# itsdfish/DifferentialEvolutionMCMC.jl

Measured on AMD Instinct MI355X. Metric: particle-updates/sec (proposal+loglike+accept) at D=32, N=1e5, higher is better.
Workload: dtype f64; 1 GPU; cfg3: MvNormal full-Sigma D=32, N=100000 obs, n_groups=256x1, Np=256, sampler defaults, schedule=two_colour, loglike=direct; particles_per_gpu=65536, parallelism=groups sharded x1, one all-gather per migration

## Files before the change

### differentialevolutionmcmc.jl_amd/csrc/demc_kernels.hpp

```cpp
#pragma once
#include <type_traits>
#include "demc_device.hpp"

namespace demc {

enum Family : int {
    FAM_GAUSSIAN = 0, FAM_MVN_ISO = 1, FAM_MVN_FULL = 2, FAM_BINOMIAL = 3, FAM_HIER_BINOMIAL = 4,
    FAM_HIER_GAUSSIAN = 5, FAM_LBA = 6, FAM_LNR = 7, FAM_RASTRIGIN = 8, FAM_USER = 100
};
enum Mode : int { MODE_STEP = 0, MODE_IDENT = 1 };

struct DimTab {
    double lo, hi;
    double a, b;
    double c;
    int kind, ref;
};

struct DimSeg {
    int start, pad;
    DimTab t;
    double pad2;
};
constexpr int kMaxDimSeg = 16;
// ... 1453 lines not shown
                        if (c0 < d) a_ = fma(tr[c0] - xb0, y0, a_);
                        if (c1 < d) a_ = fma(tr[c1] - xb1, y1, a_);
                        if (p.sx)
                            s_ = fma(y1, sx1, y0 * sx0);
                        else {
                            const int qr = q_lo + pass * ppp + wrow0 + pr;
                            if (qr < q_hi) {
                                double* yrow = STREAM ? ybuf + (size_t)(qr - q_lo) * p.dpad
                                                      : p.Ypad + ((size_t)g * Np + p.a_lo + qr) * p.dpad;
                                if (c0 < p.dpad) yrow[c0] = y0;
                                if (c1 < p.dpad) yrow[c1] = y1;
                            }
                        }
                        a_ = subgroup_sum(a_, 16);
                        s_ = subgroup_sum(s_, 16);
                        if (row == 0) {
                            tr[D] = a_;
                            tr[D + 1] = s_;
                        }
                    }
                }
                __builtin_amdgcn_fence(__ATOMIC_RELEASE, "wavefront");
                __builtin_amdgcn_wave_barrier();
                aux = th[D];
                S = th[D + 1];
            } else
            for (int k = sl; 2 * k < d; k += lpp) {
                const int c0 = 2 * k, c1 = 2 * k + 1;
                double y0 = 0.0, y1 = 0.0;
                const double* ainv_g = ld_ainv ? (const double*)ainv_s : p.Ainv;
                if (p.Ainv) {
                    if (c1 < d) {
#pragma unroll 4
                        for (int j = 0; j < d; ++j) {
                            const double t = th[j] - xb_s[j];
                            y0 = fma(ainv_g[j * d + c0], t, y0);
                            y1 = fma(ainv_g[j * d + c1], t, y1);
                        }
                    } else
                        for (int j = 0; j < d; ++j) y0 = fma(ainv_g[j * d + c0], th[j] - xb_s[j], y0);
                } else {
                    y0 = th[c0] - xb_s[c0];
                    if (c1 < d) y1 = th[c1] - xb_s[c1];
                }
                aux = fma(th[c0] - xb_s[c0], y0, aux);
                if (c1 < d) aux = fma(th[c1] - xb_s[c1], y1, aux);
                if (p.sx) {
                    S = fma(y0, p.sx[c0], S);
                    if (c1 < d) S = fma(y1, p.sx[c1], S);
                } else if (valid) {
                    double* yrow = STREAM ? ybuf + (size_t)srow * p.dpad : p.Ypad + slot * p.dpad;
                    yrow[c0] = y0;
                    if (c1 < p.dpad) yrow[c1] = (c1 < d) ? y1 : 0.0;
                }
            }
            if (!p.sx && valid && !PREP_MFMA && !STREAM)
                for (int c = 2 * ((d + 1) / 2) + sl; c < p.dpad; c += lpp) p.Ypad[slot * p.dpad + c] = 0.0;
            if (!PREP_MFMA) {
                aux = group_sum(aux, lpp, s_gsum);
                S = group_sum(S, lpp, s_gsum);
            }
        }

        if (pass == DEMC_STAMP_PASS || n_pass == 1) DEMC_STAMP(7);
        if (FUSE_OBS) {
            __builtin_amdgcn_fence(__ATOMIC_RELEASE, "wavefront");
            __builtin_amdgcn_wave_barrier();
            if (lpp > 64) __syncthreads();
            S = group_sum(obs_range_sum(p, scr + srow * scr_stride, sl, p.N, lpp), lpp, s_gsum);
        }

        if (!p.fuse_accept) {
            if (sl == 0 && valid) {
                p.prop_prior[slot] = prior;
                p.prop_oob[slot] = oob ? 1 : 0;
                p.prop_adj[slot] = adj;
                if (FUSE_PREP) {
                    p.aux[slot] = aux;
                    if (p.sx) p.partial[slot] = S;
                }
                if (!PLAIN && p.trace) {
                    p.tr_idx[slot * 4 + 0] = kind;
                    p.tr_idx[slot * 4 + 1] = i0;
                    p.tr_idx[slot * 4 + 2] = i1;
                    p.tr_idx[slot * 4 + 3] = i2;
                }
            }
            __builtin_amdgcn_fence(__ATOMIC_RELEASE, "wavefront");
            __builtin_amdgcn_wave_barrier();
            if (lpp > 64 && use_scr) __syncthreads();
            continue;
        }

        if (STREAM) {
            if (sl == 0 && valid) {
                double* tr = scr + srow * scr_stride;
                tr[D] = aux; tr[D + 2] = prior; tr[D + 3] = (double)oob; tr[D + 4] = adj; tr[D + 5] = u_acc;
                if (!PLAIN && p.trace && wr_hbm) {
                    p.tr_idx[slot * 4 + 0] = kind; p.tr_idx[slot * 4 + 1] = i0;
                    p.tr_idx[slot * 4 + 2] = i1; p.tr_idx[slot * 4 + 3] = i2;
                }
            }
            continue;
        }
        if (pass == DEMC_STAMP_PASS || n_pass == 1) DEMC_STAMP(8);
        finish_particle(valid, pl, slot, pt, srow, prior, oob, adj, aux, S, u_acc, kind, i0, i1, i2);
        __builtin_amdgcn_fence(__ATOMIC_RELEASE, "wavefront");
        __builtin_amdgcn_wave_barrier();
        if (lpp > 64 && use_scr) __syncthreads();
        if (pass == DEMC_STAMP_PASS || n_pass == 1) DEMC_STAMP(9);
    }
    if (STREAM) {
        __syncthreads();
        DEMC_STAMP(16);
        const int n_act = q_hi - q_lo;
        {
            const int nw = WG / 64;
            const int nt = xt_hi - xt_lo, per_w = (nt + nw - 1) / nw;
            const int t_lo = wave * per_w < nt ? wave * per_w : nt, t_hi = t_lo + per_w < nt ? t_lo + per_w : nt;
            lds_ptr outw = (lds_ptr)(part_l + (size_t)wave * p.st_nact_max);
            if (p.st_x_lds)
                cross_stage<lds_cptr>((lds_cptr)ybuf, p.dpad, n_act, (lds_cptr)xs, t_lo, t_hi, p.st_chunk_tiles, outw, lane);
            else
                cross_stage<glb_cptr>((lds_cptr)ybuf, p.dpad, n_act, (glb_cptr)(p.Xf + (size_t)xt_lo * (p.dpad >> 2) * 64), t_lo, t_hi,
                                      p.n_tiles - xt_lo, outw, lane);
        }
        __syncthreads();
        DEMC_STAMP(17);
        const unsigned epoch = (unsigned)(step + 1);
        unsigned long long* gran = p.st_gran + (((size_t)(step & 1) * p.n_groups + gi) * p.st_C) * p.st_nact_max * 2;
        if (tid < n_act) {
            double v = 0.0;
            for (int wv = 0; wv < WG / 64; ++wv) v += part_l[(size_t)wv * p.st_nact_max + tid];
            unsigned long long* mine = gran + ((size_t)c_idx * p.st_nact_max + tid) * 2;
            store_granule(mine, epoch, (unsigned)__double2loint(v));
            store_granule(mine + 1, epoch, (unsigned)__double2hiint(v));
        }
        DEMC_STAMP(18);
        {
            const int tot = p.st_C * n_act * 2;
            unsigned spins = 0;
            for (;;) {
                int ok = 1;
                for (int e = tid; e < tot; e += WG) {
                    const int cc = e / (2 * n_act), r = e - cc * 2 * n_act;
                    const unsigned long long x = load_granule(gran + (size_t)cc * p.st_nact_max * 2 + r);
                    ok &= (unsigned)(x >> 32) == epoch;
                    part_c[(size_t)cc * p.st_nact_max * 2 + r] = (unsigned)x;
                }
                if (__syncthreads_and(ok)) break;
                if (++spins > (1u << 22)) {
                    if (tid == 0) *p.st_err = 1u;
                    break;
                }
                __builtin_amdgcn_s_sleep(2);
            }
        }
        DEMC_STAMP(19);
        if (tid < n_act) {
            double S = 0.0;
            for (int cc = 0; cc < p.st_C; ++cc) {
                const unsigned* h2 = part_c + ((size_t)cc * p.st_nact_max + tid) * 2;
                S += __hiloint2double((int)h2[1], (int)h2[0]);
            }
            scr[tid * scr_stride + D + 1] = S;
        }
        __syncthreads();
        for (int pass = 0; pass < n_pass; ++pass) {
            const int q = q_lo + pass * ppp + sub;
            const bool valid = q < q_hi;
            const int pl = p.a_lo + (valid ? q : q_lo);
            const size_t slot = (size_t)g * Np + pl;
            const int srow = pass * ppp + sub;
            const double* tr = scr + (valid ? srow : 0) * scr_stride;
            finish_particle(valid, pl, slot, rows + (size_t)pl * D, valid ? srow : 0, tr[D + 2], (int)tr[D + 3], tr[D + 4], tr[D],
                            tr[D + 1], tr[D + 5], 0, -1, -1, -1);
        }
        DEMC_STAMP(20);
    }
    if (RES) __syncthreads();
    DEMC_STAMP(10);
    }
}

#define DEMC_K1_PHASE_INSTANCES(X) \
    X(256, false, TAIL_NONE, false, 0, false) X(256, false, TAIL_PREP, false, 0, false) \
    X(256, false, TAIL_PREP_MFMA, false, 0, false) X(256, false, TAIL_OBS, false, 0, false) \
    X(256, true, TAIL_NONE, false, 0, false) X(256, true, TAIL_PREP, false, 0, false) \
    X(256, true, TAIL_PREP_MFMA, false, 0, false) X(256, true, TAIL_OBS, false, 0, false) \
    X(256, true, TAIL_NONE, false, 1, false) X(256, true, TAIL_PREP, false, 1, false) \
    X(256, true, TAIL_PREP_MFMA, false, 1, false) X(256, true, TAIL_OBS, false, 1, false) \
    X(512, false, TAIL_NONE, false, 0, false) X(512, false, TAIL_PREP, false, 0, false) \
    X(512, false, TAIL_PREP_MFMA, false, 0, false) X(512, false, TAIL_OBS, false, 0, false) \
    X(256, true, TAIL_NONE, false, 2, false) X(256, true, TAIL_PREP, false, 2, false) \
    X(256, true, TAIL_PREP_MFMA, false, 2, false) X(256, true, TAIL_OBS, false, 2, false) \
    X(256, false, TAIL_NONE, false, 1, false) X(256, false, TAIL_PREP, false, 1, false) \
    X(256, false, TAIL_PREP_MFMA, false, 1, false) X(256, false, TAIL_OBS, false, 1, false) \
    X(256, false, TAIL_NONE, false, 2, false) X(256, false, TAIL_PREP, false, 2, false) \
    X(256, false, TAIL_PREP_MFMA, false, 2, false) X(256, false, TAIL_OBS, false, 2, false)
#define DEMC_K1_RES_INSTANCES(X) \
    X(256, true, TAIL_NONE, true, 0, false) X(256, true, TAIL_PREP, true, 0, false) \
    X(256, true, TAIL_PREP_MFMA, true, 0, false) X(256, true, TAIL_OBS, true, 0, false) \
    X(512, true, TAIL_NONE, true, 0, false) X(512, true, TAIL_PREP, true, 0, false) \
    X(512, true, TAIL_PREP_MFMA, true, 0, false) X(512, true, TAIL_OBS, true, 0, false) \
    X(256, true, TAIL_NONE, true, 1, false) X(256, true, TAIL_PREP, true, 1, false) \
    X(256, true, TAIL_PREP_MFMA, true, 1, false) X(256, true, TAIL_OBS, true, 1, false) \
    X(512, true, TAIL_NONE, true, 1, false) X(512, true, TAIL_PREP, true, 1, false) \
    X(512, true, TAIL_PREP_MFMA, true, 1, false) X(512, true, TAIL_OBS, true, 1, false) \
    X(256, true, TAIL_NONE, true, 2, false) X(256, true, TAIL_PREP, true, 2, false) \
    X(256, true, TAIL_PREP_MFMA, true, 2, false) X(256, true, TAIL_OBS, true, 2, false) \
    X(512, true, TAIL_NONE, true, 2, false) X(512, true, TAIL_PREP, true, 2, false) \
    X(512, true, TAIL_PREP_MFMA, true, 2, false) X(512, true, TAIL_OBS, true, 2, false)
#define DEMC_K1_STREAM_INSTANCES(X) \
    X(256, true, TAIL_PREP, true, 0, true) X(256, true, TAIL_PREP_MFMA, true, 0, true) \
    X(256, true, TAIL_PREP, true, 1, true) X(256, true, TAIL_PREP_MFMA, true, 1, true) \
    X(256, true, TAIL_PREP, true, 2, true) X(256, true, TAIL_PREP_MFMA, true, 2, true) \
    X(512, true, TAIL_PREP, true, 0, true) X(512, true, TAIL_PREP_MFMA, true, 0, true) \
    X(512, true, TAIL_PREP, true, 1, true) X(512, true, TAIL_PREP_MFMA, true, 1, true) \
    X(512, true, TAIL_PREP, true, 2, true) X(512, true, TAIL_PREP_MFMA, true, 2, true)
#ifdef DEMC_K1_EXTERN
#define DEMC_X_(...) extern template __global__ void k_propose<__VA_ARGS__>(KParams);
DEMC_K1_PHASE_INSTANCES(DEMC_X_)
DEMC_K1_RES_INSTANCES(DEMC_X_)
DEMC_K1_STREAM_INSTANCES(DEMC_X_)
#undef DEMC_X_
#endif

template <int KS, int MT>
__global__ __launch_bounds__(256, 2) void k_cross_mfma(KParams p, const double* __restrict__ Ypad, int dpad, int k0,
                                                       const double* __restrict__ Xf, int n_tiles, int n_chunks,
                                                       int part0) {
    const int lane = threadIdx.x & 63, wave = threadIdx.x >> 6;
    const int chunk = blockIdx.x % n_chunks;
    const int ptile = blockIdx.x / n_chunks;
    const int n_prop = p.n_groups * p.n_act;
    const int q0 = (ptile * 4 + wave) * (MT * 16);
    const int ksx = dpad >> 2;

    double a[MT][KS];
#pragma unroll
    for (int mt = 0; mt < MT; ++mt) {
        const int q = q0 + mt * 16 + (lane & 15);
        const bool ok = q < n_prop;
        const size_t slot = ok ? (size_t)slot_of(p, q) : 0;
        const double* yrow = Ypad + slot * dpad + k0 + (lane >> 4);
#pragma unroll
        for (int ks = 0; ks < KS; ++ks) {
            const double v = yrow[4 * ks];
            a[mt][ks] = ok ? v : 0.0;
        }
    }
    d4 acc[MT];
#pragma unroll
    for (int mt = 0; mt < MT; ++mt) acc[mt] = (d4){0.0, 0.0, 0.0, 0.0};

    const int per = (n_tiles + n_chunks - 1) / n_chunks;
    const int t0 = chunk * per, t1 = (t0 + per < n_tiles) ? t0 + per : n_tiles;
    const size_t tstride = (size_t)ksx * 64;
    const double* xb = Xf + (size_t)(k0 >> 2) * 64 + lane;
    double b0[KS], b1[KS];
    {
        const double* x = xb + (size_t)(t0 < t1 ? t0 : n_tiles) * tstride;
#pragma unroll
        for (int ks = 0; ks < KS; ++ks) b0[ks] = x[ks * 64];
    }
    for (int t = t0; t < t1; t += 2) {
        {
            const double* x = xb + (size_t)(t + 1 < t1 ? t + 1 : n_tiles) * tstride;
#pragma unroll
            for (int ks = 0; ks < KS; ++ks) b1[ks] = x[ks * 64];
        }
#pragma unroll
        for (int ks = 0; ks < KS; ++ks)
#pragma unroll
            for (int mt = 0; mt < MT; ++mt)
                acc[mt] = __builtin_amdgcn_mfma_f64_16x16x4f64(a[mt][ks], b0[ks], acc[mt], 0, 0, 0);
        {
            const double* x = xb + (size_t)(t + 2 < t1 ? t + 2 : n_tiles) * tstride;
#pragma unroll
            for (int ks = 0; ks < KS; ++ks) b0[ks] = x[ks * 64];
        }
#pragma unroll
        for (int ks = 0; ks < KS; ++ks)
#pragma unroll
            for (int mt = 0; mt < MT; ++mt)
                acc[mt] = __builtin_amdgcn_mfma_f64_16x16x4f64(a[mt][ks], b1[ks], acc[mt], 0, 0, 0);
    }
#pragma unroll
    for (int mt = 0; mt < MT; ++mt)
#pragma unroll
        for (int r = 0; r < 4; ++r) {
            double v = acc[mt][r];
            v += __shfl_xor(v, 1);
            v += __shfl_xor(v, 2);
            v += __shfl_xor(v, 4);
            v += __shfl_xor(v, 8);
            const int q = q0 + mt * 16 + (lane >> 4) + 4 * r;
            if ((lane & 15) == 0 && q < n_prop) p.partial[(size_t)(part0 + chunk) * p.P + slot_of(p, q)] = v;
        }
}
#define DEMC_CROSS_INSTANCES(X) X(1, 4) X(2, 4) X(4, 4) X(8, 4) X(16, 4)

template <int DP>
__global__ __launch_bounds__(256) void k_direct_mvn(KParams p, int n_chunks, unsigned long long* __restrict__ clk) {
    int pblock = blockIdx.x, chunk = blockIdx.y;
    if ((n_chunks & 7) == 0) {
        const unsigned lin = blockIdx.y * gridDim.x + blockIdx.x, xcd = lin & 7u, j = lin >> 3;
        chunk = (int)((j / gridDim.x) * 8u + xcd);
        pblock = (int)(j % gridDim.x);
    }
    const int q = pblock * 256 + threadIdx.x;
    const int n_prop = p.n_groups * p.n_act;
    const bool ok = q < n_prop;
    const size_t slot = ok ? (size_t)slot_of(p, q) : 0;
    double m[DP];
    const double* mrow = p.Ypad + slot * p.dpad;
#pragma unroll
    for (int k = 0; k < DP; ++k) m[k] = (ok && k < p.d) ? mrow[k] : 0.0;
    const long long per = (p.N + n_chunks - 1) / n_chunks;
    const long long i0 = chunk * per, i1 = (i0 + per < p.N) ? i0 + per : p.N;
    double acc[4] = {0.0, 0.0, 0.0, 0.0};
    const double* z = p.data + i0 * DP;
    for (long long i = i0; i < i1; ++i, z += DP) {
#pragma unroll
        for (int k = 0; k < DP; k += 4) {
#pragma unroll
            for (int e = 0; e < 4; ++e) {
                const double r = z[k + e] - m[k + e];
                acc[e] = fma(r, r, acc[e]);
            }
        }
    }
    if (ok) p.partial[(size_t)chunk * p.P + slot] = (acc[0] + acc[1]) + (acc[2] + acc[3]);
    if (clk) {
        const unsigned long long t1 = __builtin_amdgcn_s_memtime(), r1 = __builtin_amdgcn_s_memrealtime();
        const unsigned xcc = __builtin_amdgcn_s_getreg(20 | (3 << 11)) & 15u;
        const unsigned hwid = __builtin_amdgcn_s_getreg(4 | (31 << 11));
        if (threadIdx.x == 0) {
            const size_t wg = (size_t)blockIdx.y * gridDim.x + blockIdx.x;
            clk[3 * wg] = t1;
            clk[3 * wg + 1] = r1;
            clk[3 * wg + 2] = (xcc << 8) | ((hwid >> 8) & 0xffu);
        }
    }
}
#define DEMC_DIRECT_INSTANCES(X) X(8) X(16) X(32) X(64)

#ifndef DEMC_DEVICE_HELPERS_ONLY
__global__ __launch_bounds__(256) void k_obs_loglike(KParams p, int n_chunks) {
    constexpr int kTabPhi = kPhiIntervals * kPhiRow, kTabErfcx = kLogPhiRows * kLogPhiRow;
    __shared__ double s_tab[kTabPhi > kTabErfcx ? kTabPhi : kTabErfcx];
    if (p.family == FAM_LBA) {
        for (int i = threadIdx.x; i < kTabPhi; i += 256) s_tab[i] = kPhiTable[i];
        __syncthreads();
    } else if (p.family == FAM_LNR) {
        for (int i = threadIdx.x; i < kTabErfcx; i += 256) s_tab[i] = kLogPhiTable[i];
        __syncthreads();
    }
    const int q = blockIdx.x * 256 + threadIdx.x;
    const int n_prop = p.n_groups * p.n_act;
    const int chunk = blockIdx.y;
    if (q >= n_prop) return;
    const size_t slot = (size_t)slot_of(p, q);
    const double* th = p.prop + slot * p.D;
    const long long per = (p.N + n_chunks - 1) / n_chunks;
    const long long i0 = chunk * per, i1 = (i0 + per < p.N) ? i0 + per : p.N;
    double acc;
    if (p.family == FAM_LBA)
        acc = p.n_acc == 3 ? lba_range_sum<3>(p, th, i0, i1, 1, s_tab)
              : p.n_acc == 2 ? lba_range_sum<2>(p, th, i0, i1, 1, s_tab) : lba_range_sum<0>(p, th, i0, i1, 1, s_tab);
    else if (p.family == FAM_LNR)
        acc = lnr_range_sum(p, th, i0, i1, 1, s_tab);
    else
        acc = obs_range_sum(p, th, i0, i1, 1);
    p.partial[(size_t)chunk * p.P + slot] = acc;
}
#endif

#ifndef DEMC_DEVICE_HELPERS_ONLY
template <int NA>
__global__ __launch_bounds__(256, 2) void k_lba_wave(KParams p, int n_chunks, unsigned long long* __restrict__ clk) {
    __shared__ double s_tab[kPhiIntervals * kPhiRow];
    for (int i = threadIdx.x; i < kPhiIntervals * kPhiRow; i += 256) s_tab[i] = kPhiTable[i];
    __syncthreads();
    const int lane = threadIdx.x & 63, wave = __builtin_amdgcn_readfirstlane(threadIdx.x >> 6);
    const int q = blockIdx.x * 4 + wave;
    const int n_prop = p.n_groups * p.n_act;
    const int chunk = blockIdx.y;
    if (q >= n_prop) return;
    const size_t slot = (size_t)slot_of(p, q);
    const double* th = p.prop + slot * p.D;
    const int na = NA > 0 ? NA : p.n_acc;
    double nu[8], nuS[8];
#pragma unroll
    for (int a = 0; a < 8; ++a) {
        nu[a] = a < na ? th[a] : 0.0;
        nuS[a] = kPhiS * nu[a];
    }
    const double A = th[na], kk = th[na + 1], tau = th[na + 2], b = A + kk, inv_A = 1.0 / A;
    const double kS = kPhiS * kk, bS = kPhiS * b, inv_SA = inv_A * (1.0 / kPhiS);
    double pneg = 1.0;
#pragma unroll
    for (int a = 0; a < (NA > 0 ? NA : 8); ++a)
        if (a < na) {
            double qq, Ph;
            phiS_Phi_table(s_tab, -nuS[a], qq, Ph);
            pneg *= Ph;
        }
    const double inv_norm = 1.0 / (1.0 - pneg);
    constexpr long long kStep = 64LL * kLbaBatch;
    const long long n_steps = (p.N + kStep - 1) / kStep, per = (n_steps + n_chunks - 1) / n_chunks;
    const long long i0 = (long long)chunk * per * kStep, i1r = i0 + per * kStep, i1 = i1r < p.N ? i1r : p.N;
    double acc = 0.0;
    long long base = i0;
    for (; base + kStep <= i1; base += kStep) {
        double cc[kLbaBatch], rr[kLbaBatch];
#pragma unroll
        for (int j = 0; j < kLbaBatch; ++j) {
            cc[j] = p.data[base + 64LL * j + lane];
            rr[j] = p.data2[base + 64LL * j + lane];
        }
        double prod = 1.0;
#pragma unroll
        for (int j = 0; j < kLbaBatch; ++j)
            prod *= lba_trial<NA, double>(s_tab, na, nu, nuS, kS, bS, tau, inv_A, inv_SA, inv_norm, cc[j], rr[j]);
        if (__builtin_expect(!(prod < 1e300), 0)) {
            double s2 = 0.0;
#pragma unroll 1
            for (int j = 0; j < kLbaBatch; ++j)
                s2 += log(lba_trial<NA, double>(s_tab, na, nu, nuS, kS, bS, tau, inv_A, inv_SA, inv_norm, cc[j], rr[j]));
            acc += s2;
        } else
            acc += log(prod);
    }
#pragma unroll 1
    for (long long i = base + lane; i < i1; i += 64)
        acc += log(lba_trial<NA, double>(s_tab, na, nu, nuS, kS, bS, tau, inv_A, inv_SA, inv_norm, p.data[i], p.data2[i]));
    acc = subgroup_sum(acc, 64);
    if (lane == 0) p.partial[(size_t)chunk * p.P + slot] = acc;
    if (clk) {
        const unsigned long long t1 = __builtin_amdgcn_s_memtime(), r1 = __builtin_amdgcn_s_memrealtime();
        const unsigned xcc = __builtin_amdgcn_s_getreg(20 | (3 << 11)) & 15u, hwid = __builtin_amdgcn_s_getreg(4 | (31 << 11));
        if (threadIdx.x == 0) {
            const size_t wg = (size_t)blockIdx.y * gridDim.x + blockIdx.x;
            clk[3 * wg] = t1;
            clk[3 * wg + 1] = r1;
            clk[3 * wg + 2] = (xcc << 8) | ((hwid >> 8) & 0xffu);
        }
    }
}
#define DEMC_LBA_WAVE_INSTANCES(X) X(3) X(2) X(0)
#endif

#ifndef DEMC_DEVICE_HELPERS_ONLY
__global__ __launch_bounds__(256) void k_hier_loglike(KParams p) {
    __shared__ double s_part[4];
    const int tid = threadIdx.x, lane = tid & 63;
    const int q = blockIdx.x;
    const size_t slot = (size_t)slot_of(p, q);
    const double* th = p.prop + slot * p.D;
    const long long S = p.N;
    double acc = 0.0;
    if (p.family == FAM_HIER_BINOMIAL) {
        const double mu0 = th[0], n = p.c0;
        const double* lgc = p.data + S;
        for (long long s = tid; s < S; s += 256) {
            const double eta = mu0 + th[2 + s], k = p.data[s];
            acc += lgc[s] - n * softplus_fast(-eta) - (n - k) * eta;
        }
    } else {
        const double mu0 = th[0], sg = th[2 + S];
        const int n = p.d;
        const double lsg = log(sg), isg = 1.0 / sg;
        for (long long s = tid; s < S; s += 256) {
            const double mu = mu0 + th[2 + s];
            double l = 0.0;
            for (int i = 0; i < n; ++i) {
                const double z = (p.data[s * n + i] - mu) * isg;
                l += -(z * z + kLog2Pi) / 2.0 - lsg;
            }
            acc += l;
        }
    }
    for (int o = 32; o > 0; o >>= 1) acc += __shfl_xor(acc, o);
    if (lane == 0) s_part[tid >> 6] = acc;
    __syncthreads();
    if (tid == 0) p.partial[slot] = (s_part[0] + s_part[1]) + (s_part[2] + s_part[3]);
}
#endif

__device__ inline double sum_partials(const KParams& p, size_t slot, int sl, int lpp) {
    double s = 0.0;
    if (lpp > 64) {
        for (int c = 0; c < p.n_partials; ++c) s += p.partial[(size_t)c * p.P + slot];
        return s;
    }
    for (int c = sl; c < p.n_partials; c += lpp) s += p.partial[(size_t)c * p.P + slot];
    return subgroup_sum(s, lpp);
}
__device__ inline double finalize_loglike(const KParams& p, size_t slot, double s) {
    double sg = 0.0;
    if (p.family == FAM_MVN_ISO) sg = p.prop[slot * p.D + p.d];
    if (p.family == FAM_GAUSSIAN) sg = p.prop[slot * p.D + 1];
    return loglike_from_stats(p, s, p.aux[slot], sg);
}

#ifndef DEMC_DEVICE_HELPERS_ONLY
__global__ __launch_bounds__(256) void k_accept_store(KParams p) {
    const int tid = threadIdx.x;
    const int lpp = p.lpp3, ppp = 256 / lpp;
    const int sub = tid / lpp, sl = tid % lpp;
    const int n_prop = p.n_groups * p.n_act;
    const int q = blockIdx.x * ppp + sub;
    const bool valid = q < n_prop;
    int g = 0, pl = 0;
    const size_t slot = valid ? (size_t)slot_of(p, q, g, pl) : 0;
    const int D = p.D;
    int acc = 0;
    double w_new = 0.0;
    const double s_sum = sum_partials(p, slot, sl, lpp);
    if (sl == 0 && valid) {
        const double w = p.weight[slot];
        const bool oob = p.prop_oob[slot] != 0;
        double wp;
        if (p.fitness_kind == 1)
            wp = oob ? (p.update_kind == 1 ? -INFINITY : INFINITY) : finalize_loglike(p, slot, s_sum);
        else
            wp = oob ? -INFINITY : p.prop_prior[slot] + finalize_loglike(p, slot, s_sum);
        const uint32_t eslot = (uint32_t)(p.group_offset + g) * (uint32_t)p.Np + (uint32_t)pl;
        const U4 ra = draw_block(p.seed, S_PART, p.sweep, (uint64_t)p.iter, eslot, 3);
        const double u_acc = replayed(p.rp_part, slot * 5 + 4, u53(ra.x, ra.y));
        acc = decide(p, u_acc, wp, w, p.prop_adj[slot]);
        w_new = acc ? wp : w;
        if (acc) p.weight[slot] = wp;
        if (p.trace) {
            p.tr_w[slot] = wp;
            p.tr_acc[slot] = (unsigned char)acc;
        }
        if (p.store_row >= 0) {
            const size_t hrow = (size_t)p.store_row * p.P + slot;
            if (p.update_kind == 0 && p.mode == MODE_STEP) {
                p.acc_hist[hrow] = (unsigned char)acc;
                p.lp_hist[hrow] = w_new;
            }
            p.id_hist[hrow] = (int)p.id[slot];
        }
    }
    if (lpp > 64) {
        __shared__ int s_acc;
        if (tid == 0) s_acc = acc;
        __syncthreads();
        acc = s_acc;
    } else
        acc = (int)subgroup_bcast<0>((uint32_t)acc, lpp, (tid & 63) & ~(lpp - 1));
    if (!valid) return;
    double* trow = p.theta + slot * D;
    const double* prow = p.prop + slot * D;
    double* hrow = (p.store_row >= 0) ? p.hist + ((size_t)p.store_row * p.P + slot) * p.hist_ld : nullptr;
    if (!acc && !hrow) return;
    for (int k = sl; 2 * k < D; k += lpp)
        for (int e = 0; e < 2; ++e) {
            const int j = 2 * k + e;
            if (j < D) {
                double v;
                if (acc) {
                    v = prow[j];
                    trow[j] = v;
                } else
                    v = trow[j];
                if (hrow) hrow[j] = v;
            }
        }
}
#endif


#ifndef DEMC_DEVICE_HELPERS_ONLY
__global__ __launch_bounds__(256) void k_mig_pack(KParams p, double* __restrict__ rows) {
    extern __shared__ double lds[];
    __shared__ double s_red[4];
    __shared__ int s_redi[4];
    __shared__ int s_bad, s_pick;
    const int tid = threadIdx.x, g = blockIdx.x, Np = p.Np, D = p.D;
    const double* gw = p.weight + (size_t)g * Np;
    double* cdf = lds;
    double* ctot = lds + Np;
    double m = INFINITY;
    int am = 0x7fffffff, bad = 0;
    if (tid == 0) s_bad = 0;
    for (int i = tid; i < Np; i += 256) {
        const double w = gw[i];
        if (!(w > -INFINITY)) bad = 1;
        if (w < m) { m = w; am = i; }
    }
    for (int o = 32; o > 0; o >>= 1) {
        const double m2 = __shfl_xor(m, o);
        const int a2 = __shfl_xor(am, o);
        if (m2 < m || (m2 == m && a2 < am)) { m = m2; am = a2; }
    }
    __syncthreads();
    if (bad) s_bad = 1;
    if ((tid & 63) == 0) { s_red[tid >> 6] = m; s_redi[tid >> 6] = am; }
    __syncthreads();
    for (int k = 0; k < 4; ++k) {
        const double m2 = s_red[k];
        const int a2 = s_redi[k];
        if (m2 < m || (m2 == m && a2 < am)) { m = m2; am = a2; }
    }
    if (s_bad || !(m < INFINITY)) {
        if (tid == 0) s_pick = am < Np ? am : 0;
    } else {
        const int n_chunk = (Np + 15) >> 4;
        for (int i = tid; i < Np; i += 256) cdf[i] = exp(m - gw[i]);
        __syncthreads();
        for (int c = tid; c < n_chunk; c += 256) {
            double v[16];
#pragma unroll
            for (int k = 0; k < 16; ++k) v[k] = (c * 16 + k < Np) ? cdf[c * 16 + k] : 0.0;
            const double pre = chunk16_prefix(v);
#pragma unroll
            for (int k = 0; k < 16; ++k)
                if (c * 16 + k < Np) cdf[c * 16 + k] = v[k];
            ctot[c] = pre;
        }
        __syncthreads();
        if (tid == 0) {
            double off = 0.0;
            for (int c = 0; c < n_chunk; ++c) {
                const double t = ctot[c];
                ctot[c] = off;
                off = off + t;
            }
        }
        __syncthreads();
        for (int i = tid; i < Np; i += 256) cdf[i] = ctot[i >> 4] + cdf[i];
        __syncthreads();
// ... 125 lines not shown
```

Measured before the change: 5.201 million particle-updates/s.

## Split D=32 direct MVN loglike across waves with double-buffered scalar loads

For DP=32, each wave now handles a 16-dimension slice for two proposals per lane, and the partial sums of the two slices are combined through shared memory. Data rows are fetched with explicit s_load_dwordx16 into SGPRs, double-buffered so the next row loads while the current one is computed. Each row load is shared by the whole wave as a scalar broadcast, which cuts vector memory traffic and register pressure. This relies on inline asm and manual waitcnt handling, and adds a block-wide sync plus a shared-memory reduction.

```diff
diff --git a/differentialevolutionmcmc.jl_amd/csrc/demc_kernels.hpp b/differentialevolutionmcmc.jl_amd/csrc/demc_kernels.hpp
--- a/differentialevolutionmcmc.jl_amd/csrc/demc_kernels.hpp
+++ b/differentialevolutionmcmc.jl_amd/csrc/demc_kernels.hpp
@@ -1779,6 +1779,99 @@
 #define DEMC_CROSS_INSTANCES(X) X(1, 4) X(2, 4) X(4, 4) X(8, 4) X(16, 4)
 
 template <int DP>
+__device__ __forceinline__ void direct_mvn_rows(const KParams& p, int pblock, int chunk, int n_chunks) {
+    const int q = pblock * 256 + threadIdx.x;
+    const bool ok = q < p.n_groups * p.n_act;
+    const size_t slot = ok ? (size_t)slot_of(p, q) : 0;
+    double m[DP];
+    const double* mrow = p.Ypad + slot * p.dpad;
+#pragma unroll
+    for (int k = 0; k < DP; ++k) m[k] = (ok && k < p.d) ? mrow[k] : 0.0;
+    const long long per = (p.N + n_chunks - 1) / n_chunks;
+    const long long i0 = chunk * per, i1 = (i0 + per < p.N) ? i0 + per : p.N;
+    double acc[4] = {0.0, 0.0, 0.0, 0.0};
+    const double* z = p.data + i0 * DP;
+    for (long long i = i0; i < i1; ++i, z += DP) {
+#pragma unroll
+        for (int k = 0; k < DP; k += 4) {
+#pragma unroll
+            for (int e = 0; e < 4; ++e) {
+                const double r = z[k + e] - m[k + e];
+                acc[e] = fma(r, r, acc[e]);
+            }
+        }
+    }
+    if (ok) p.partial[(size_t)chunk * p.P + slot] = (acc[0] + acc[1]) + (acc[2] + acc[3]);
+}
+
+typedef int zs16 __attribute__((ext_vector_type(16)));
+typedef double zd8 __attribute__((ext_vector_type(8)));
+__device__ __forceinline__ void zslice_ask(zs16& lo, zs16& hi, const double* row) {
+    asm volatile("s_load_dwordx16 %0, %2, 0x0\n\ts_load_dwordx16 %1, %2, 0x40" : "=&s"(lo), "=&s"(hi) : "s"(row) : "memory");
+    __builtin_amdgcn_sched_barrier(0);
+}
+__device__ __forceinline__ void zslice_wait(zs16& lo, zs16& hi) {
+    asm volatile("s_waitcnt lgkmcnt(0)" : "+s"(lo), "+s"(hi));
+    __builtin_amdgcn_sched_barrier(0);
+}
+__device__ __forceinline__ void zslice_fma(const zs16& lo, const zs16& hi, const double (&m0)[16], const double (&m1)[16],
+                                           double (&a0)[2], double (&a1)[2]) {
+    const zd8 zl = __builtin_bit_cast(zd8, lo), zh = __builtin_bit_cast(zd8, hi);
+#pragma unroll
+    for (int k = 0; k < 16; ++k) {
+        const double z = k < 8 ? zl[k & 7] : zh[k & 7];
+        const double r0 = z - m0[k], r1 = z - m1[k];
+        a0[k & 1] = fma(r0, r0, a0[k & 1]);
+        a1[k & 1] = fma(r1, r1, a1[k & 1]);
+    }
+}
+__device__ __forceinline__ void direct_mvn_slices(const KParams& p, int pblock, int chunk, int n_chunks) {
+    __shared__ double s_other[256];
+    const int lane = threadIdx.x & 63, wave = __builtin_amdgcn_readfirstlane(threadIdx.x >> 6);
+    const int s = wave >> 1, h = wave & 1;
+    const int n_prop = p.n_groups * p.n_act;
+    const int t0 = h * 128 + lane, t1 = t0 + 64;
+    const bool ok0 = pblock * 256 + t0 < n_prop, ok1 = pblock * 256 + t1 < n_prop;
+    const size_t slot0 = ok0 ? (size_t)slot_of(p, pblock * 256 + t0) : 0, slot1 = ok1 ? (size_t)slot_of(p, pblock * 256 + t1) : 0;
+    double m0[16], m1[16];
+    const double *mrow0 = p.Ypad + slot0 * p.dpad + 16 * s, *mrow1 = p.Ypad + slot1 * p.dpad + 16 * s;
+#pragma unroll
+    for (int k = 0; k < 16; ++k) {
+        m0[k] = (ok0 && 16 * s + k < p.d) ? mrow0[k] : 0.0;
+        m1[k] = (ok1 && 16 * s + k < p.d) ? mrow1[k] : 0.0;
+    }
+    const long long per = (p.N + n_chunks - 1) / n_chunks;
+    const long long i0 = chunk * per, i1 = (i0 + per < p.N) ? i0 + per : p.N;
+    const int n = (int)(i1 - i0);
+    double a0[2] = {0.0, 0.0}, a1[2] = {0.0, 0.0};
+    if (n > 0) {
+        const double* z = p.data + i0 * 32 + 16 * s;
+        zs16 alo, ahi, blo, bhi;
+        zslice_ask(alo, ahi, z);
+        for (int left = n; left >= 2; left -= 2, z += 64) {
+            zslice_wait(alo, ahi);
+            zslice_ask(blo, bhi, z + 32);
+            zslice_fma(alo, ahi, m0, m1, a0, a1);
+            zslice_wait(blo, bhi);
+            zslice_ask(alo, ahi, left > 2 ? z + 64 : z + 32);
+            zslice_fma(blo, bhi, m0, m1, a0, a1);
+        }
+        zslice_wait(alo, ahi);
+        if (n & 1) zslice_fma(alo, ahi, m0, m1, a0, a1);
+    }
+    const double sum0 = a0[0] + a0[1], sum1 = a1[0] + a1[1];
+    if (s == 1) {
+        s_other[t0] = sum0;
+        s_other[t1] = sum1;
+    }
+    __syncthreads();
+    if (s == 0) {
+        if (ok0) p.partial[(size_t)chunk * p.P + slot0] = sum0 + s_other[t0];
+        if (ok1) p.partial[(size_t)chunk * p.P + slot1] = sum1 + s_other[t1];
+    }
+}
+
+template <int DP>
 __global__ __launch_bounds__(256) void k_direct_mvn(KParams p, int n_chunks, unsigned long long* __restrict__ clk) {
     int pblock = blockIdx.x, chunk = blockIdx.y;
     if ((n_chunks & 7) == 0) {
@@ -1786,29 +1879,10 @@
         chunk = (int)((j / gridDim.x) * 8u + xcd);
         pblock = (int)(j % gridDim.x);
     }
-    const int q = pblock * 256 + threadIdx.x;
-    const int n_prop = p.n_groups * p.n_act;
-    const bool ok = q < n_prop;
-    const size_t slot = ok ? (size_t)slot_of(p, q) : 0;
-    double m[DP];
-    const double* mrow = p.Ypad + slot * p.dpad;
-#pragma unroll
-    for (int k = 0; k < DP; ++k) m[k] = (ok && k < p.d) ? mrow[k] : 0.0;
-    const long long per = (p.N + n_chunks - 1) / n_chunks;
-    const long long i0 = chunk * per, i1 = (i0 + per < p.N) ? i0 + per : p.N;
-    double acc[4] = {0.0, 0.0, 0.0, 0.0};
-    const double* z = p.data + i0 * DP;
-    for (long long i = i0; i < i1; ++i, z += DP) {
-#pragma unroll
-        for (int k = 0; k < DP; k += 4) {
-#pragma unroll
-            for (int e = 0; e < 4; ++e) {
-                const double r = z[k + e] - m[k + e];
-                acc[e] = fma(r, r, acc[e]);
-            }
-        }
-    }
-    if (ok) p.partial[(size_t)chunk * p.P + slot] = (acc[0] + acc[1]) + (acc[2] + acc[3]);
+    if constexpr (DP == 32)
+        direct_mvn_slices(p, pblock, chunk, n_chunks);
+    else
+        direct_mvn_rows<DP>(p, pblock, chunk, n_chunks);
     if (clk) {
         const unsigned long long t1 = __builtin_amdgcn_s_memtime(), r1 = __builtin_amdgcn_s_memrealtime();
         const unsigned xcc = __builtin_amdgcn_s_getreg(20 | (3 << 11)) & 15u;
```

Measured after the change: 5.423 million particle-updates/s, median of 6. 1.04x the previous value.
